# may-/joeys2t

Hardware: AMD Instinct MI355X
Metric: audio frames/sec (train step, 80-mel, 15 s utt, bs32 per GPU) (higher is better)
Workload: dtype bf16; 1 GPU; configs/librispeech_100h.yaml ASR train step on synthetic 16 kHz waveforms; global_batch=32, frames_per_utt=1498, encoder_len=375, lengths=fixed 15 s, vocab=5000, batch_multiplier=1, parallelism=dp1, launch=hipGraph replay

## Files before the change

### include/joeys2t_hip.h

```cpp
#ifndef JOEYS2T_HIP_H
#define JOEYS2T_HIP_H

#include <stdint.h>

#ifdef __cplusplus
extern "C" {
#endif

typedef void* js2t_stream;

enum { JS2T_F32 = 0, JS2T_BF16 = 1, JS2T_FP8_E4M3 = 2  };
enum { JS2T_ACT_NONE = 0, JS2T_ACT_RELU = 1, JS2T_ACT_GELU = 2, JS2T_ACT_SWISH = 3, JS2T_ACT_TANH = 4, JS2T_ACT_HARDSWISH = 5 };
enum { JS2T_OK = 0, JS2T_ERR_INVALID = -1, JS2T_ERR_LAUNCH = -2, JS2T_ERR_UNSUPPORTED = -3 };

int js2t_abi_version(void);
const char* js2t_last_error(void);

typedef struct js2t_gemm_desc {
  int32_t M, N, K;
  int32_t batch, batch_inner;
  int32_t dtype_ab, dtype_c;
  int32_t trans_a, trans_b;
  const void* A; int64_t lda, a_stride_o, a_stride_i;
  const void* B; int64_t ldb, b_stride_o, b_stride_i;
// ... 188 lines not shown
               float log_floor, js2t_stream stream);

int js2t_cmvn_stats(const float* feat, const int64_t* frame_off, int32_t U, int32_t F, float* mean, float* istd,
                    float* fill, int32_t norm_means, int32_t norm_vars, int64_t max_frames, js2t_stream stream);
int64_t js2t_cmvn_stats_workspace(int32_t U, int32_t F);
int js2t_cmvn_stats_ws(const float* feat, const int64_t* frame_off, int32_t U, int32_t F, float* mean, float* istd, float* fill,
                       int32_t norm_means, int32_t norm_vars, int64_t max_frames, double* workspace, js2t_stream stream);

int js2t_feature_finalize(const float* feat, const int64_t* frame_off, const float* mean, const float* istd,
                          const float* fill, const int32_t* masks, void* out, int out_dt, int64_t U, int64_t Tmax,
                          int32_t F, float pad_value, js2t_stream stream);
int js2t_feature_finalize_crop(const float* feat, const int64_t* frame_off, const float* mean, const float* istd,
                               const float* fill, const int32_t* masks, void* out, int out_dt, int64_t U, int64_t Tmax,
                               int32_t F, float pad_value, const int64_t* crop_t, js2t_stream stream);

int js2t_feature_transform(float* feat, const int64_t* frame_off, int32_t U, int32_t F, const float* mean, const float* istd,
                           const float* fill, const int32_t* masks, int32_t n_freq, int32_t n_time, js2t_stream stream);

typedef struct js2t_ctx_s* js2t_ctx;
enum {
  JS2T_CTX_DETERMINISTIC = 0,
  JS2T_CTX_GEMM_P192_MODE = 1,
  JS2T_CTX_GEMM_P192_RING = 2,
  JS2T_CTX_GEMM_WG256_MODE = 3,
  JS2T_CTX_GEMM_PANEL_MODE = 4,
  JS2T_CTX_NKEYS = 5
};
js2t_ctx js2t_ctx_create(void);
void js2t_ctx_destroy(js2t_ctx ctx);
int js2t_ctx_set(js2t_ctx ctx, int32_t key, int32_t value);
// ... 83 lines not shown
```

### joeys2t_amd/csrc/fbank.hip

```cpp
#include "common.hpp"

namespace {

constexpr int FB_WAVES = 4;
constexpr int FB_MAX_FFT = 1024;

__device__ __forceinline__ int find_utt(const int64_t* __restrict__ frame_off, int U, int64_t f) {
  int lo = 0, hi = U;
  while (hi - lo > 1) {
    const int mid = (lo + hi) >> 1;
    if (frame_off[mid] <= f) lo = mid; else hi = mid;
  }
  return lo;
}

__global__ __launch_bounds__(256) void fbank_kernel(const float* __restrict__ wave, const int64_t* __restrict__ sample_off,
                                                    const int64_t* __restrict__ frame_off, int U,
                                                    const float* __restrict__ window, const float* __restrict__ tw_re,
                                                    const float* __restrict__ tw_im, const int32_t* __restrict__ mel_start,
                                                    const int32_t* __restrict__ mel_len, const int32_t* __restrict__ mel_woff,
                                                    const float* __restrict__ mel_w, float* __restrict__ out, int win_len,
                                                    int shift, int n_fft, int log2_fft, int n_mel, float scale,
                                                    float preemph, float log_floor) {
  __shared__ float sre[FB_WAVES][FB_MAX_FFT];
// ... 83 lines not shown
struct cplx { float re, im; };
__device__ __forceinline__ cplx cmul(cplx a, cplx b) { return {a.re * b.re - a.im * b.im, a.re * b.im + a.im * b.re}; }
__device__ __forceinline__ void bfly(cplx& a, cplx& b, cplx w) {
  const cplx d = {a.re - b.re, a.im - b.im};
  a = {a.re + b.re, a.im + b.im};
  b = cmul(d, w);
}
__device__ __forceinline__ void bfly1(cplx& a, cplx& b) {
  const cplx d = {a.re - b.re, a.im - b.im};
  a = {a.re + b.re, a.im + b.im};
  b = d;
}
__device__ __forceinline__ int rev3(int v) { return ((v & 1) << 2) | (v & 2) | ((v >> 2) & 1); }

constexpr int FB5_T1 = 72, FB5_T2 = 9;
constexpr int FB5_MELW = 2048;
__global__ __launch_bounds__(256) void fbank512_kernel(const float* __restrict__ wave, const int64_t* __restrict__ sample_off,
                                                       const int64_t* __restrict__ frame_off, int U,
                                                       const float* __restrict__ window, const float* __restrict__ tw_re,
                                                       const float* __restrict__ tw_im, const int32_t* __restrict__ mel_start,
                                                       const int32_t* __restrict__ mel_len, const int32_t* __restrict__ mel_woff,
                                                       const float* __restrict__ mel_w, float* __restrict__ out, int win_len,
                                                       int shift, int n_mel, float scale, float preemph, float log_floor) {
  __shared__ float2 simg[FB_WAVES][8 * FB5_T1];
  __shared__ float spw[FB_WAVES][256];
  __shared__ float smw[FB5_MELW];
  const int lane = threadIdx.x & 63, w = threadIdx.x >> 6;
  float2* img = simg[w];
  float* pw = spw[w];
  const int n_mel_w = mel_woff[n_mel - 1] + mel_len[n_mel - 1];
  const bool mw_lds = n_mel_w <= FB5_MELW;
  if (mw_lds)
    for (int i = threadIdx.x; i < n_mel_w; i += 256) smw[i] = mel_w[i];
  __syncthreads();
  int mst[2], mln[2], mwo[2];
#pragma unroll
  for (int q = 0; q < 2; ++q) {
    const int mb = lane + 64 * q;
    mst[q] = mb < n_mel ? mel_start[mb] : 0;
    mln[q] = mb < n_mel ? mel_len[mb] : 0;
    mwo[q] = mb < n_mel ? mel_woff[mb] : 0;
  }
  auto tw = [&](int t) -> cplx { return {tw_re[t], tw_im[t]}; };
  const int r = lane & 7;
  cplx w1[4], w2[2], w3, w4[4], w5[2], w6;
#pragma unroll
  for (int j = 0; j < 4; ++j) w1[j] = tw(lane + 64 * j);
#pragma unroll
  for (int j = 0; j < 2; ++j) w2[j] = tw(2 * (lane + 64 * j));
  w3 = tw(4 * lane);
#pragma unroll
  for (int m = 0; m < 4; ++m) w4[m] = tw(8 * (r + 8 * m));
#pragma unroll
  for (int m = 0; m < 2; ++m) w5[m] = tw(16 * (r + 8 * m));
  w6 = tw(32 * r);
  const cplx c8[4] = {{1.f, 0.f}, {0.70710678118654752f, -0.70710678118654752f}, {0.f, -1.f}, {-0.70710678118654752f, -0.70710678118654752f}};
  float win[8];
#pragma unroll
  for (int j = 0; j < 8; ++j) win[j] = lane + 64 * j < win_len ? window[lane + 64 * j] : 0.f;
  const int64_t total = frame_off[U];
  const int64_t n_waves = (int64_t)gridDim.x * FB_WAVES, per = (total + n_waves - 1) / n_waves;
  const int64_t f0 = ((int64_t)blockIdx.x * FB_WAVES + w) * per, f1 = min(total, f0 + per);
  int u = f0 < total ? find_utt(frame_off, U, f0) : 0;
  int64_t u_end = f0 < total ? frame_off[u + 1] : 0, u_beg = f0 < total ? frame_off[u] : 0, s_off = f0 < total ? sample_off[u] : 0;
  auto frame_ptr = [&](int64_t f) -> const float* {
    while (f >= u_end) {
      ++u;
      u_beg = u_end;
      u_end = frame_off[u + 1];
      s_off = sample_off[u];
    }
    return wave + s_off + (f - u_beg) * shift;
  };
  float nxt[8];
  if (f0 < f1) {
    const float* x0 = frame_ptr(f0);
#pragma unroll
    for (int j = 0; j < 8; ++j) nxt[j] = lane + 64 * j < win_len ? x0[lane + 64 * j] : 0.f;
  }
  for (int64_t f = f0; f < f1; ++f) {
    float cur[8], prv[8], sum = 0.f;
#pragma unroll
    for (int j = 0; j < 8; ++j) {
      cur[j] = nxt[j] * scale;
      sum += cur[j];
    }
    if (f + 1 < f1) {
      const float* xn = frame_ptr(f + 1);
#pragma unroll
      for (int j = 0; j < 8; ++j) nxt[j] = lane + 64 * j < win_len ? xn[lane + 64 * j] : 0.f;
    }
#pragma unroll
    for (int j = 0; j < 8; ++j) {
      const float up = __int_as_float(__builtin_amdgcn_update_dpp(0, __float_as_int(cur[j]), 0x138 , 0xf, 0xf, false));
      const int edge = j == 0 ? __builtin_amdgcn_readfirstlane(__float_as_int(cur[0]))
                              : __builtin_amdgcn_readlane(__float_as_int(cur[j > 0 ? j - 1 : 0]), 63);
      prv[j] = lane == 0 ? __int_as_float(edge) : up;
    }
    const float mean = wave_sum(sum) / (float)win_len;
    cplx a[8];
#pragma unroll
    for (int j = 0; j < 8; ++j) a[j] = {lane + 64 * j < win_len ? ((cur[j] - mean) - preemph * (prv[j] - mean)) * win[j] : 0.f, 0.f};
#pragma unroll
    for (int j = 0; j < 4; ++j) bfly(a[j], a[j + 4], w1[j]);
#pragma unroll
    for (int hlf = 0; hlf < 8; hlf += 4)
#pragma unroll
      for (int j = 0; j < 2; ++j) bfly(a[hlf + j], a[hlf + j + 2], w2[j]);
#pragma unroll
    for (int j = 0; j < 8; j += 2) bfly(a[j], a[j + 1], w3);
#pragma unroll
    for (int j = 0; j < 8; ++j) img[j * FB5_T1 + lane] = make_float2(a[j].re, a[j].im);
    asm volatile("s_waitcnt lgkmcnt(0)" ::: "memory");
    const int jp = lane >> 3;
#pragma unroll
    for (int m = 0; m < 8; ++m) {
      const float2 v = img[jp * FB5_T1 + r + 8 * m];
      a[m] = {v.x, v.y};
    }
    asm volatile("s_waitcnt lgkmcnt(0)" ::: "memory");
#pragma unroll
    for (int m = 0; m < 4; ++m) bfly(a[m], a[m + 4], w4[m]);
#pragma unroll
    for (int hlf = 0; hlf < 8; hlf += 4)
#pragma unroll
      for (int m = 0; m < 2; ++m) bfly(a[hlf + m], a[hlf + m + 2], w5[m]);
#pragma unroll
    for (int m = 0; m < 8; m += 2) bfly(a[m], a[m + 1], w6);
#pragma unroll
    for (int m = 0; m < 8; ++m) img[(8 * jp + m) * FB5_T2 + r] = make_float2(a[m].re, a[m].im);
    asm volatile("s_waitcnt lgkmcnt(0)" ::: "memory");
#pragma unroll
    for (int q = 0; q < 8; ++q) {
      const float2 v = img[lane * FB5_T2 + q];
      a[q] = {v.x, v.y};
    }
#pragma unroll
    for (int q = 0; q < 4; ++q) bfly(a[q], a[q + 4], c8[q]);
#pragma unroll
    for (int hlf = 0; hlf < 8; hlf += 4) {
      bfly1(a[hlf], a[hlf + 2]);
      bfly(a[hlf + 1], a[hlf + 3], c8[2]);
    }
#pragma unroll
    for (int q = 0; q < 8; q += 2) bfly1(a[q], a[q + 1]);
    const int mm = lane & 7, base = 8 * rev3(mm) + rev3(jp);
#pragma unroll
    for (int q = 0; q < 8; q += 2) pw[64 * rev3(q) + base] = a[q].re * a[q].re + a[q].im * a[q].im;
    asm volatile("s_waitcnt lgkmcnt(0)" ::: "memory");
#pragma unroll
    for (int q = 0; q < 2; ++q) {
      const int mb = lane + 64 * q;
      if (mb < n_mel) {
        const float* wt = mw_lds ? smw + mwo[q] : mel_w + mwo[q];
        const float* pp = pw + mst[q];
        float e0 = 0.f, e1 = 0.f, e2 = 0.f, e3 = 0.f;
        int k = 0;
        for (; k + 4 <= mln[q]; k += 4) {
          e0 += pp[k] * wt[k];
          e1 += pp[k + 1] * wt[k + 1];
          e2 += pp[k + 2] * wt[k + 2];
          e3 += pp[k + 3] * wt[k + 3];
        }
        for (; k < mln[q]; ++k) e0 += pp[k] * wt[k];
        out[f * n_mel + mb] = __logf(fmaxf((e0 + e1) + (e2 + e3), log_floor));
      }
    }
    for (int mb = lane + 128; mb < n_mel; mb += 64) {
      const int st = mel_start[mb], ln = mel_len[mb];
      const float* wt = mel_w + mel_woff[mb];
      float e = 0.f;
      for (int k = 0; k < ln; ++k) e += pw[st + k] * wt[k];
      out[f * n_mel + mb] = __logf(fmaxf(e, log_floor));
    }
    asm volatile("s_waitcnt lgkmcnt(0)" ::: "memory");
  }
}

constexpr int CM_GROUPS = 12;
constexpr int CM_SPLIT = 8;
__global__ void cmvn_partial_kernel(const float* __restrict__ feat, const int64_t* __restrict__ frame_off, int F, double* __restrict__ part,
                                    int64_t max_frames) {
  extern __shared__ double sh[];
  const int u = blockIdx.x, p = blockIdx.y;
  const int64_t t0 = frame_off[u], T = max_frames > 0 ? min(frame_off[u + 1] - t0, max_frames) : frame_off[u + 1] - t0;
  const int64_t per = (T + CM_SPLIT - 1) / CM_SPLIT, ta = min(T, p * per), tb = min(T, ta + per);
  const int c = threadIdx.x % F, gi = threadIdx.x / F;
  double s = 0.0, q = 0.0;
// ... 101 lines not shown
    float v = t < crop ? pad_value : 0.f;
    if (t < T) {
      v = feat[(t0 + t) * F + c];
      if (mean) v = (v - mean[u * F + c]) * istd[u * F + c];
      if (masks) {
        const int32_t* m = masks + u * 8;
        const bool hit = (m[1] > 0 && c >= m[0] && c < m[0] + m[1]) || (m[3] > 0 && c >= m[2] && c < m[2] + m[3]) ||
                         (m[5] > 0 && t >= m[4] && t < m[4] + m[5]) || (m[7] > 0 && t >= m[6] && t < m[6] + m[7]);
        if (hit) v = fill[u];
      }
    }
    io<TO>::st(out + i, v);
  }
}

__global__ void feature_transform_kernel(float* __restrict__ feat, const int64_t* __restrict__ frame_off, int F,
                                         const float* __restrict__ mean, const float* __restrict__ istd,
                                         const float* __restrict__ fill, const int32_t* __restrict__ masks, int n_freq, int n_time) {
  const int u = blockIdx.y;
  const int64_t t0 = frame_off[u], n = (frame_off[u + 1] - t0) * F;
  const int32_t* m = masks ? masks + (int64_t)u * 2 * (n_freq + n_time) : nullptr;
  for (int64_t i = blockIdx.x * (int64_t)blockDim.x + threadIdx.x; i < n; i += (int64_t)gridDim.x * blockDim.x) {
    const int64_t t = i / F;
    const int c = (int)(i - t * F);
    float v = feat[t0 * F + i];
    if (mean) v = (v - mean[(int64_t)u * F + c]) * istd[(int64_t)u * F + c];
    if (m) {
      bool hit = false;
      for (int k = 0; k < n_freq; ++k) hit = hit || (m[2 * k + 1] > 0 && c >= m[2 * k] && c < m[2 * k] + m[2 * k + 1]);
      for (int k = n_freq; k < n_freq + n_time; ++k) hit = hit || (m[2 * k + 1] > 0 && t >= m[2 * k] && t < m[2 * k] + m[2 * k + 1]);
// ... 95 lines not shown
  int64_t g = (U * Tmax * F + 255) / 256;
  if (g > 8192) g = 8192;
  if (out_dt == JS2T_F32)
    hipLaunchKernelGGL((feature_finalize_kernel<float>), dim3((unsigned)g), dim3(256), 0, (hipStream_t)stream, feat, frame_off,
                       mean, istd, fill, masks, (float*)out, U, Tmax, F, pad_value, crop_t);
  else if (out_dt == JS2T_BF16)
    hipLaunchKernelGGL((feature_finalize_kernel<uint16_t>), dim3((unsigned)g), dim3(256), 0, (hipStream_t)stream, feat,
                       frame_off, mean, istd, fill, masks, (uint16_t*)out, U, Tmax, F, pad_value, crop_t);
  else {
    js2t_set_error("feature_finalize: bad dtype");
    return JS2T_ERR_INVALID;
  }
  JS2T_LAUNCH_CHECK();
  return JS2T_OK;
}
```

### joeys2t_amd/data_augmentation.py

```python
import ctypes as C
import math
from typing import Optional, Sequence

import numpy as np
import torch

from joeys2t_amd import ops
from joeys2t_amd._lib import check, lib

_p, _stream = ops._p, ops._stream


class SpecAugment:

    def __init__(self, freq_mask_n: int = 2, freq_mask_f: int = 27, time_mask_n: int = 2, time_mask_t: int = 40,
                 time_mask_p: float = 1.0, mask_value: Optional[float] = None):
        self.freq_mask_n, self.freq_mask_f = freq_mask_n, freq_mask_f
        self.time_mask_n, self.time_mask_t, self.time_mask_p = time_mask_n, time_mask_t, time_mask_p
        self.mask_value = mask_value

    @property
    def slots(self):
        return max(2, self.freq_mask_n), max(2, self.time_mask_n)

# ... 21 lines not shown

    def __repr__(self):
        return (f"{self.__class__.__name__}(freq_mask_n={self.freq_mask_n}, freq_mask_f={self.freq_mask_f}, "
                f"time_mask_n={self.time_mask_n}, time_mask_t={self.time_mask_t}, time_mask_p={self.time_mask_p})")


class CMVN:

    def __init__(self, norm_means: bool = True, norm_vars: bool = True, before: bool = True):
        self.norm_means, self.norm_vars, self.before = norm_means, norm_vars, before

    def __repr__(self):
        return f"{self.__class__.__name__}(norm_means={self.norm_means}, norm_vars={self.norm_vars}, before={self.before})"


def finalize_features(feat: torch.Tensor, frame_off: torch.Tensor, frames: Sequence[int], *, cmvn: Optional[CMVN],
                      specaugment: Optional[SpecAugment], out_dtype=torch.float32, pad_value: float = 1.0,
                      max_length: Optional[int] = None, masks_dev: Optional[torch.Tensor] = None, t_pad: Optional[int] = None,
                      crop_t: Optional[torch.Tensor] = None):
    ops._dev(feat, frame_off)
    U, F = len(frames), feat.shape[1]
    dev = feat.device
    eff = [min(int(t), max_length) if max_length else int(t) for t in frames]
    Tmax = max(eff) if t_pad is None else int(t_pad)
    mean = istd = fill = masks = None
    fused = ((cmvn is None or cmvn.before) and (specaugment is None or specaugment.fused) and
             not (specaugment is not None and cmvn is None and specaugment.mask_value is None))
    if not fused:
        if masks_dev is not None or crop_t is not None:
            raise NotImplementedError("graph-replayed batches (masks_dev / crop_t) take the fused front-end: CMVN before SpecAugment, "
                                      "at most two masks of each kind")
        return _finalize_general(feat, frame_off, eff, cmvn, specaugment, out_dtype, pad_value, max_length, Tmax)
    if cmvn is not None:
        mean = torch.empty((U, F), dtype=torch.float32, device=dev)
        istd = torch.empty((U, F), dtype=torch.float32, device=dev)
        fill = torch.empty((U, ), dtype=torch.float32, device=dev)
        ws = torch.empty((int(lib().js2t_cmvn_stats_workspace(C.c_int32(U), C.c_int32(F))), ), dtype=torch.float64, device=dev)
        check(lib().js2t_cmvn_stats_ws(_p(feat), _p(frame_off), C.c_int32(U), C.c_int32(F), _p(mean), _p(istd), _p(fill),
                                       C.c_int32(int(cmvn.norm_means)), C.c_int32(int(cmvn.norm_vars)),
                                       C.c_int64(int(max_length) if max_length else 0), _p(ws), _stream()),
              "js2t_cmvn_stats_ws")
    if specaugment is not None:
        if masks_dev is not None:
            masks = masks_dev
        else:
            m = np.stack([specaugment.draw(t, F) for t in eff])
            masks = torch.from_numpy(m).to(dev)
        if specaugment.mask_value is not None:
            fill = torch.full((U, ), float(specaugment.mask_value), dtype=torch.float32, device=dev)
    out = torch.empty((U, Tmax, F), dtype=out_dtype, device=dev)
    check(lib().js2t_feature_finalize_crop(_p(feat), _p(frame_off), _p(mean), _p(istd), _p(fill), _p(masks), _p(out),
                                           ops.dt_code(out), C.c_int64(U), C.c_int64(Tmax), C.c_int32(F), C.c_float(pad_value),
                                           _p(crop_t), _stream()), "js2t_feature_finalize")
    return out, eff


def _stats(feat, frame_off, U, F, norm_means, norm_vars, max_length):
    dev = feat.device
    mean = torch.empty((U, F), dtype=torch.float32, device=dev)
    istd = torch.empty((U, F), dtype=torch.float32, device=dev)
    fill = torch.empty((U, ), dtype=torch.float32, device=dev)
    check(lib().js2t_cmvn_stats(_p(feat), _p(frame_off), C.c_int32(U), C.c_int32(F), _p(mean), _p(istd), _p(fill), C.c_int32(int(norm_means)),
                                C.c_int32(int(norm_vars)), C.c_int64(int(max_length) if max_length else 0), _stream()), "js2t_cmvn_stats")
    return mean, istd, fill

# ... 30 lines not shown
```

### joeys2t_amd/helpers_for_audio.py

```python
import ctypes as C
from pathlib import Path
from typing import Dict, List, Optional, Sequence, Tuple

import numpy as np
import torch

from joeys2t_amd import ops
from joeys2t_amd._lib import check, lib

_p, _stream = ops._p, ops._stream


def get_n_frames(wave_length: int, sample_rate: int) -> int:
    duration_ms = int(wave_length / sample_rate * 1000)
    return int(1 + (duration_ms - 25) / 10)


def _mel(f):
    return 1127.0 * np.log(1.0 + np.asarray(f, dtype=np.float64) / 700.0)


class FbankExtractor:

    def __init__(self, device, sample_rate: int = 16000, n_mel_bins: int = 80, frame_length_ms: float = 25.0,
# ... 25 lines not shown
            starts.append(st), lens.append(ln), woffs.append(len(wts))
            wts.extend(banks[m, st:st + ln].astype(np.float32).tolist())
        dev = self.device
        self.window = torch.tensor(window, dtype=torch.float32, device=dev)
        self.tw_re = torch.tensor(np.cos(ang), dtype=torch.float32, device=dev)
        self.tw_im = torch.tensor(-np.sin(ang), dtype=torch.float32, device=dev)
        self.mel_start = torch.tensor(starts, dtype=torch.int32, device=dev)
        self.mel_len = torch.tensor(lens, dtype=torch.int32, device=dev)
        self.mel_woff = torch.tensor(woffs, dtype=torch.int32, device=dev)
        self.mel_w = torch.tensor(wts if wts else [0.0], dtype=torch.float32, device=dev)
        self._plans = {}

    def n_frames(self, n_samples: int) -> int:
        return 0 if n_samples < self.win_len else 1 + (n_samples - self.win_len) // self.shift

    def batch(self, wave: torch.Tensor, n_samples: Sequence[int], sample_off: Optional[Sequence[int]] = None):
        ops._dev(wave)
        if wave.dtype != torch.float32 or not wave.is_contiguous():
            raise ops.Js2tError("fbank: waveform buffer must be contiguous float32")
        U = len(n_samples)
        if sample_off is None:
            stride = wave.shape[-1] if wave.dim() == 2 else 0
            sample_off = [u * stride for u in range(U)]
        if wave.numel() < max(o + n for o, n in zip(sample_off, n_samples)):
            raise ops.Js2tError("fbank: waveform buffer shorter than sample_off + n_samples")
        key = (tuple(int(n) for n in n_samples), tuple(int(o) for o in sample_off))
        plan = self._plans.get(key)
        if plan is None:
            frames = [self.n_frames(int(n)) for n in n_samples]
            foff = np.concatenate([[0], np.cumsum(frames)]).astype(np.int64)
            plan = (frames, torch.tensor(list(sample_off), dtype=torch.int64, device=self.device),
                    torch.tensor(foff, dtype=torch.int64, device=self.device), int(foff[-1]))
            if len(self._plans) > 64:
                self._plans.clear()
            self._plans[key] = plan
        frames, d_soff, d_foff, total = plan
        return self.batch_tables(wave, d_soff, d_foff, U, total), d_foff, frames

    def batch_tables(self, wave: torch.Tensor, d_soff: torch.Tensor, d_foff: torch.Tensor, U: int, total_cap: int) -> torch.Tensor:
        ops._dev(wave, d_soff, d_foff)
        total = int(total_cap)
        feat = torch.empty((total, self.n_mel), dtype=torch.float32, device=self.device)
        check(lib().js2t_fbank(_p(wave), _p(d_soff), _p(d_foff), C.c_int32(U), C.c_int64(total), _p(self.window),
                               _p(self.tw_re), _p(self.tw_im), _p(self.mel_start), _p(self.mel_len), _p(self.mel_woff),
                               _p(self.mel_w), _p(feat), C.c_int32(self.win_len), C.c_int32(self.shift), C.c_int32(self.n_fft),
                               C.c_int32(self.n_mel), C.c_float(2.0**15), C.c_float(self.preemph),
                               C.c_float(float(np.finfo(np.float32).eps)), _stream()), "js2t_fbank")
        return feat


_extractors: Dict[Tuple, FbankExtractor] = {}


def get_extractor(device, sample_rate: int = 16000, n_mel_bins: int = 80) -> FbankExtractor:
    key = (str(device), int(sample_rate), int(n_mel_bins))
    if key not in _extractors:
        _extractors[key] = FbankExtractor(device, sample_rate, n_mel_bins)
# ... 29 lines not shown
```

### joeys2t_amd/tokenizers.py

```python
import re
from typing import List, Optional, Sequence, Tuple, Union

import torch

from joeys2t_amd.data_augmentation import CMVN, SpecAugment, finalize_features
from joeys2t_amd.helpers_for_audio import get_extractor


class SpeechProcessor:
    def __init__(self, level: str = "frame", num_freq: int = 80, normalize: bool = False, max_length: int = -1,
                 min_length: int = -1, sample_rate: int = 16000, **kwargs):
        self.level = level
        self.num_freq = num_freq
        self.normalize = normalize
        self.max_length = max_length
        self.min_length = min_length
        self.sample_rate = sample_rate
        self.specaugment: Optional[SpecAugment] = SpecAugment(**kwargs["specaugment"]) if "specaugment" in kwargs else None
        self.cmvn: Optional[CMVN] = CMVN(**kwargs["cmvn"]) if "cmvn" in kwargs else None

    def keep_mask(self, frames: Sequence[int], is_train: bool) -> List[bool]:
        keep = []
        for t in frames:
            ok = not (self.min_length > t > 0)
            if ok and 0 < self.max_length < t and is_train:
                ok = False
            keep.append(ok)
        return keep

    def draw_masks(self, frames: Sequence[int]):
        import numpy as np
        eff = [min(int(t), self.max_length) if self.max_length > 0 else int(t) for t in frames]
        return np.stack([self.specaugment.draw(t, self.num_freq) for t in eff])

    def batch_from_waveforms(self, wave: torch.Tensor, n_samples: Sequence[int], is_train: bool = False,
                             out_dtype=torch.float32, sample_off: Optional[Sequence[int]] = None,
                             masks_dev: Optional[torch.Tensor] = None) -> Tuple[torch.Tensor, List[int]]:
        ex = get_extractor(wave.device, self.sample_rate, self.num_freq)
        feat, frame_off, frames = ex.batch(wave, n_samples, sample_off)
        sa = self.specaugment if is_train else None
        return finalize_features(feat, frame_off, frames, cmvn=self.cmvn, specaugment=sa, out_dtype=out_dtype,
                                 max_length=self.max_length if self.max_length > 0 else None, masks_dev=masks_dev)

    def batch_from_tables(self, wave: torch.Tensor, d_soff: torch.Tensor, d_foff: torch.Tensor, n_utts: int, t_pad: int,
                          crop_t: torch.Tensor, is_train: bool = True, out_dtype=torch.float32,
                          masks_dev: Optional[torch.Tensor] = None) -> torch.Tensor:
        ex = get_extractor(wave.device, self.sample_rate, self.num_freq)
        feat = ex.batch_tables(wave, d_soff, d_foff, n_utts, n_utts * t_pad)
        sa = self.specaugment if is_train else None
        if sa is not None and masks_dev is None:
            raise ValueError("batch_from_tables: SpecAugment parameters must be supplied in masks_dev")
        out, _ = finalize_features(feat, d_foff, [t_pad] * n_utts, cmvn=self.cmvn, specaugment=sa, out_dtype=out_dtype,
                                   max_length=None, masks_dev=masks_dev, t_pad=t_pad, crop_t=crop_t)
        return out

    def __repr__(self):
        return (f"{self.__class__.__name__}(level={self.level}, normalize={self.normalize}, "
                f"filter_by_length=({self.min_length}, {self.max_length}), specaugment={self.specaugment}, cmvn={self.cmvn})")


_SPACE_RUNS = re.compile("[ \u3000]+")


def remove_extra_spaces(s: str) -> str:
    s = _SPACE_RUNS.sub(" ", s.replace("\u200b", ""))
    for mark in "?!,.:":
        s = s.replace(" " + mark, mark)
    return s.strip()
# ... 142 lines not shown
```

Measured before the change: 4.270 million frames/s.

## Fuse fbank with CMVN partial statistics and fold stats reduction into finalize

```diff
diff --git a/include/joeys2t_hip.h b/include/joeys2t_hip.h
--- a/include/joeys2t_hip.h
+++ b/include/joeys2t_hip.h
@@ -226,6 +226,16 @@
                                const float* fill, const int32_t* masks, void* out, int out_dt, int64_t U, int64_t Tmax,
                                int32_t F, float pad_value, const int64_t* crop_t, js2t_stream stream);
 
+int js2t_frontend_fused(const float* wave, const int64_t* sample_off, const int64_t* frame_off, int32_t U, int64_t total_frames,
+                        const float* window, const float* tw_re, const float* tw_im, const int32_t* mel_start,
+                        const int32_t* mel_len, const int32_t* mel_woff, const float* mel_w, float* out, int32_t win_len,
+                        int32_t shift, int32_t n_fft, int32_t n_mel, float scale, float preemph, float log_floor,
+                        int64_t max_frames, double* part, js2t_stream stream);
+int js2t_feature_finalize_fused(const float* feat, const int64_t* frame_off, const double* part, int32_t norm_means,
+                                int32_t norm_vars, int64_t max_frames, const float* fill, const int32_t* masks, void* out,
+                                int out_dt, int64_t U, int64_t Tmax, int32_t F, float pad_value, const int64_t* crop_t,
+                                float* mean_out, float* istd_out, float* fill_out, js2t_stream stream);
+
 int js2t_feature_transform(float* feat, const int64_t* frame_off, int32_t U, int32_t F, const float* mean, const float* istd,
                            const float* fill, const int32_t* masks, int32_t n_freq, int32_t n_time, js2t_stream stream);
 
diff --git a/joeys2t_amd/csrc/fbank.hip b/joeys2t_amd/csrc/fbank.hip
--- a/joeys2t_amd/csrc/fbank.hip
+++ b/joeys2t_amd/csrc/fbank.hip
@@ -121,7 +121,130 @@
 __device__ __forceinline__ int rev3(int v) { return ((v & 1) << 2) | (v & 2) | ((v >> 2) & 1); }
 
 constexpr int FB5_T1 = 72, FB5_T2 = 9;
+constexpr int FB5_IMG = 8 * FB5_T1;
 constexpr int FB5_MELW = 2048;
+
+struct fb5_lane {
+  cplx w1[4], w2[2], w3, w4[4], w5[2], w6;
+  float win[8];
+  int mst[2], mln[2], mwo[2];
+};
+__device__ __forceinline__ void fb5_lane_init(fb5_lane& k, int lane, const float* __restrict__ window, const float* __restrict__ tw_re,
+                                              const float* __restrict__ tw_im, const int32_t* __restrict__ mel_start,
+                                              const int32_t* __restrict__ mel_len, const int32_t* __restrict__ mel_woff, int win_len,
+                                              int n_mel) {
+#pragma unroll
+  for (int q = 0; q < 2; ++q) {
+    const int mb = lane + 64 * q;
+    k.mst[q] = mb < n_mel ? mel_start[mb] : 0;
+    k.mln[q] = mb < n_mel ? mel_len[mb] : 0;
+    k.mwo[q] = mb < n_mel ? mel_woff[mb] : 0;
+  }
+  auto tw = [&](int t) -> cplx { return {tw_re[t], tw_im[t]}; };
+  const int r = lane & 7;
+#pragma unroll
+  for (int j = 0; j < 4; ++j) k.w1[j] = tw(lane + 64 * j);
+#pragma unroll
+  for (int j = 0; j < 2; ++j) k.w2[j] = tw(2 * (lane + 64 * j));
+  k.w3 = tw(4 * lane);
+#pragma unroll
+  for (int m = 0; m < 4; ++m) k.w4[m] = tw(8 * (r + 8 * m));
+#pragma unroll
+  for (int m = 0; m < 2; ++m) k.w5[m] = tw(16 * (r + 8 * m));
+  k.w6 = tw(32 * r);
+#pragma unroll
+  for (int j = 0; j < 8; ++j) k.win[j] = lane + 64 * j < win_len ? window[lane + 64 * j] : 0.f;
+}
+
+__device__ __forceinline__ void fb5_frame(const fb5_lane& k, const float (&raw)[8], int lane, float2* img, float* pw, const float* wts, int win_len,
+                                          int n_mel, float scale, float preemph, float log_floor, float (&e)[2]) {
+  const cplx c8[4] = {{1.f, 0.f}, {0.70710678118654752f, -0.70710678118654752f}, {0.f, -1.f}, {-0.70710678118654752f, -0.70710678118654752f}};
+  const int r = lane & 7;
+  float cur[8], prv[8], sum = 0.f;
+#pragma unroll
+  for (int j = 0; j < 8; ++j) {
+    cur[j] = raw[j] * scale;
+    sum += cur[j];
+  }
+#pragma unroll
+  for (int j = 0; j < 8; ++j) {
+    const float up = __int_as_float(__builtin_amdgcn_update_dpp(0, __float_as_int(cur[j]), 0x138 , 0xf, 0xf, false));
+    const int edge = j == 0 ? __builtin_amdgcn_readfirstlane(__float_as_int(cur[0]))
+                            : __builtin_amdgcn_readlane(__float_as_int(cur[j > 0 ? j - 1 : 0]), 63);
+    prv[j] = lane == 0 ? __int_as_float(edge) : up;
+  }
+  const float mean = wave_sum(sum) / (float)win_len;
+  cplx a[8];
+#pragma unroll
+  for (int j = 0; j < 8; ++j) a[j] = {lane + 64 * j < win_len ? ((cur[j] - mean) - preemph * (prv[j] - mean)) * k.win[j] : 0.f, 0.f};
+#pragma unroll
+  for (int j = 0; j < 4; ++j) bfly(a[j], a[j + 4], k.w1[j]);
+#pragma unroll
+  for (int hlf = 0; hlf < 8; hlf += 4)
+#pragma unroll
+    for (int j = 0; j < 2; ++j) bfly(a[hlf + j], a[hlf + j + 2], k.w2[j]);
+#pragma unroll
+  for (int j = 0; j < 8; j += 2) bfly(a[j], a[j + 1], k.w3);
+#pragma unroll
+  for (int j = 0; j < 8; ++j) img[j * FB5_T1 + lane] = make_float2(a[j].re, a[j].im);
+  asm volatile("s_waitcnt lgkmcnt(0)" ::: "memory");
+  const int jp = lane >> 3;
+#pragma unroll
+  for (int m = 0; m < 8; ++m) {
+    const float2 v = img[jp * FB5_T1 + r + 8 * m];
+    a[m] = {v.x, v.y};
+  }
+  asm volatile("s_waitcnt lgkmcnt(0)" ::: "memory");
+#pragma unroll
+  for (int m = 0; m < 4; ++m) bfly(a[m], a[m + 4], k.w4[m]);
+#pragma unroll
+  for (int hlf = 0; hlf < 8; hlf += 4)
+#pragma unroll
+    for (int m = 0; m < 2; ++m) bfly(a[hlf + m], a[hlf + m + 2], k.w5[m]);
+#pragma unroll
+  for (int m = 0; m < 8; m += 2) bfly(a[m], a[m + 1], k.w6);
+#pragma unroll
+  for (int m = 0; m < 8; ++m) img[(8 * jp + m) * FB5_T2 + r] = make_float2(a[m].re, a[m].im);
+  asm volatile("s_waitcnt lgkmcnt(0)" ::: "memory");
+#pragma unroll
+  for (int q = 0; q < 8; ++q) {
+    const float2 v = img[lane * FB5_T2 + q];
+    a[q] = {v.x, v.y};
+  }
+  asm volatile("s_waitcnt lgkmcnt(0)" ::: "memory");
+#pragma unroll
+  for (int q = 0; q < 4; ++q) bfly(a[q], a[q + 4], c8[q]);
+#pragma unroll
+  for (int hlf = 0; hlf < 8; hlf += 4) {
+    bfly1(a[hlf], a[hlf + 2]);
+    bfly(a[hlf + 1], a[hlf + 3], c8[2]);
+  }
+#pragma unroll
+  for (int q = 0; q < 8; q += 2) bfly1(a[q], a[q + 1]);
+  const int mm = lane & 7, base = 8 * rev3(mm) + rev3(jp);
+#pragma unroll
+  for (int q = 0; q < 8; q += 2) pw[64 * rev3(q) + base] = a[q].re * a[q].re + a[q].im * a[q].im;
+  asm volatile("s_waitcnt lgkmcnt(0)" ::: "memory");
+#pragma unroll
+  for (int q = 0; q < 2; ++q) {
+    e[q] = 0.f;
+    if (lane + 64 * q < n_mel) {
+      const float* wt = wts + k.mwo[q];
+      const float* pp = pw + k.mst[q];
+      float e0 = 0.f, e1 = 0.f, e2 = 0.f, e3 = 0.f;
+      int i = 0;
+      for (; i + 4 <= k.mln[q]; i += 4) {
+        e0 += pp[i] * wt[i];
+        e1 += pp[i + 1] * wt[i + 1];
+        e2 += pp[i + 2] * wt[i + 2];
+        e3 += pp[i + 3] * wt[i + 3];
+      }
+      for (; i < k.mln[q]; ++i) e0 += pp[i] * wt[i];
+      e[q] = __logf(fmaxf((e0 + e1) + (e2 + e3), log_floor));
+    }
+  }
+}
+
 __global__ __launch_bounds__(256) void fbank512_kernel(const float* __restrict__ wave, const int64_t* __restrict__ sample_off,
                                                        const int64_t* __restrict__ frame_off, int U,
                                                        const float* __restrict__ window, const float* __restrict__ tw_re,
@@ -129,7 +252,7 @@
                                                        const int32_t* __restrict__ mel_len, const int32_t* __restrict__ mel_woff,
                                                        const float* __restrict__ mel_w, float* __restrict__ out, int win_len,
                                                        int shift, int n_mel, float scale, float preemph, float log_floor) {
-  __shared__ float2 simg[FB_WAVES][8 * FB5_T1];
+  __shared__ float2 simg[FB_WAVES][FB5_IMG];
   __shared__ float spw[FB_WAVES][256];
   __shared__ float smw[FB5_MELW];
   const int lane = threadIdx.x & 63, w = threadIdx.x >> 6;
@@ -140,31 +263,8 @@
   if (mw_lds)
     for (int i = threadIdx.x; i < n_mel_w; i += 256) smw[i] = mel_w[i];
   __syncthreads();
-  int mst[2], mln[2], mwo[2];
-#pragma unroll
-  for (int q = 0; q < 2; ++q) {
-    const int mb = lane + 64 * q;
-    mst[q] = mb < n_mel ? mel_start[mb] : 0;
-    mln[q] = mb < n_mel ? mel_len[mb] : 0;
-    mwo[q] = mb < n_mel ? mel_woff[mb] : 0;
-  }
-  auto tw = [&](int t) -> cplx { return {tw_re[t], tw_im[t]}; };
-  const int r = lane & 7;
-  cplx w1[4], w2[2], w3, w4[4], w5[2], w6;
-#pragma unroll
-  for (int j = 0; j < 4; ++j) w1[j] = tw(lane + 64 * j);
-#pragma unroll
-  for (int j = 0; j < 2; ++j) w2[j] = tw(2 * (lane + 64 * j));
-  w3 = tw(4 * lane);
-#pragma unroll
-  for (int m = 0; m < 4; ++m) w4[m] = tw(8 * (r + 8 * m));
-#pragma unroll
-  for (int m = 0; m < 2; ++m) w5[m] = tw(16 * (r + 8 * m));
-  w6 = tw(32 * r);
-  const cplx c8[4] = {{1.f, 0.f}, {0.70710678118654752f, -0.70710678118654752f}, {0.f, -1.f}, {-0.70710678118654752f, -0.70710678118654752f}};
-  float win[8];
-#pragma unroll
-  for (int j = 0; j < 8; ++j) win[j] = lane + 64 * j < win_len ? window[lane + 64 * j] : 0.f;
+  fb5_lane k;
+  fb5_lane_init(k, lane, window, tw_re, tw_im, mel_start, mel_len, mel_woff, win_len, n_mel);
   const int64_t total = frame_off[U];
   const int64_t n_waves = (int64_t)gridDim.x * FB_WAVES, per = (total + n_waves - 1) / n_waves;
   const int64_t f0 = ((int64_t)blockIdx.x * FB_WAVES + w) * per, f1 = min(total, f0 + per);
@@ -186,99 +286,24 @@
     for (int j = 0; j < 8; ++j) nxt[j] = lane + 64 * j < win_len ? x0[lane + 64 * j] : 0.f;
   }
   for (int64_t f = f0; f < f1; ++f) {
-    float cur[8], prv[8], sum = 0.f;
-#pragma unroll
-    for (int j = 0; j < 8; ++j) {
-      cur[j] = nxt[j] * scale;
-      sum += cur[j];
-    }
+    float raw[8], e[2];
+#pragma unroll
+    for (int j = 0; j < 8; ++j) raw[j] = nxt[j];
     if (f + 1 < f1) {
       const float* xn = frame_ptr(f + 1);
 #pragma unroll
       for (int j = 0; j < 8; ++j) nxt[j] = lane + 64 * j < win_len ? xn[lane + 64 * j] : 0.f;
     }
-#pragma unroll
-    for (int j = 0; j < 8; ++j) {
-      const float up = __int_as_float(__builtin_amdgcn_update_dpp(0, __float_as_int(cur[j]), 0x138 , 0xf, 0xf, false));
-      const int edge = j == 0 ? __builtin_amdgcn_readfirstlane(__float_as_int(cur[0]))
-                              : __builtin_amdgcn_readlane(__float_as_int(cur[j > 0 ? j - 1 : 0]), 63);
-      prv[j] = lane == 0 ? __int_as_float(edge) : up;
-    }
-    const float mean = wave_sum(sum) / (float)win_len;
-    cplx a[8];
-#pragma unroll
-    for (int j = 0; j < 8; ++j) a[j] = {lane + 64 * j < win_len ? ((cur[j] - mean) - preemph * (prv[j] - mean)) * win[j] : 0.f, 0.f};
-#pragma unroll
-    for (int j = 0; j < 4; ++j) bfly(a[j], a[j + 4], w1[j]);
-#pragma unroll
-    for (int hlf = 0; hlf < 8; hlf += 4)
-#pragma unroll
-      for (int j = 0; j < 2; ++j) bfly(a[hlf + j], a[hlf + j + 2], w2[j]);
-#pragma unroll
-    for (int j = 0; j < 8; j += 2) bfly(a[j], a[j + 1], w3);
-#pragma unroll
-    for (int j = 0; j < 8; ++j) img[j * FB5_T1 + lane] = make_float2(a[j].re, a[j].im);
-    asm volatile("s_waitcnt lgkmcnt(0)" ::: "memory");
-    const int jp = lane >> 3;
-#pragma unroll
-    for (int m = 0; m < 8; ++m) {
-      const float2 v = img[jp * FB5_T1 + r + 8 * m];
-      a[m] = {v.x, v.y};
-    }
-    asm volatile("s_waitcnt lgkmcnt(0)" ::: "memory");
-#pragma unroll
-    for (int m = 0; m < 4; ++m) bfly(a[m], a[m + 4], w4[m]);
-#pragma unroll
-    for (int hlf = 0; hlf < 8; hlf += 4)
-#pragma unroll
-      for (int m = 0; m < 2; ++m) bfly(a[hlf + m], a[hlf + m + 2], w5[m]);
-#pragma unroll
-    for (int m = 0; m < 8; m += 2) bfly(a[m], a[m + 1], w6);
-#pragma unroll
-    for (int m = 0; m < 8; ++m) img[(8 * jp + m) * FB5_T2 + r] = make_float2(a[m].re, a[m].im);
-    asm volatile("s_waitcnt lgkmcnt(0)" ::: "memory");
-#pragma unroll
-    for (int q = 0; q < 8; ++q) {
-      const float2 v = img[lane * FB5_T2 + q];
-      a[q] = {v.x, v.y};
-    }
-#pragma unroll
-    for (int q = 0; q < 4; ++q) bfly(a[q], a[q + 4], c8[q]);
-#pragma unroll
-    for (int hlf = 0; hlf < 8; hlf += 4) {
-      bfly1(a[hlf], a[hlf + 2]);
-      bfly(a[hlf + 1], a[hlf + 3], c8[2]);
-    }
-#pragma unroll
-    for (int q = 0; q < 8; q += 2) bfly1(a[q], a[q + 1]);
-    const int mm = lane & 7, base = 8 * rev3(mm) + rev3(jp);
-#pragma unroll
-    for (int q = 0; q < 8; q += 2) pw[64 * rev3(q) + base] = a[q].re * a[q].re + a[q].im * a[q].im;
-    asm volatile("s_waitcnt lgkmcnt(0)" ::: "memory");
-#pragma unroll
-    for (int q = 0; q < 2; ++q) {
-      const int mb = lane + 64 * q;
-      if (mb < n_mel) {
-        const float* wt = mw_lds ? smw + mwo[q] : mel_w + mwo[q];
-        const float* pp = pw + mst[q];
-        float e0 = 0.f, e1 = 0.f, e2 = 0.f, e3 = 0.f;
-        int k = 0;
-        for (; k + 4 <= mln[q]; k += 4) {
-          e0 += pp[k] * wt[k];
-          e1 += pp[k + 1] * wt[k + 1];
-          e2 += pp[k + 2] * wt[k + 2];
-          e3 += pp[k + 3] * wt[k + 3];
-        }
-        for (; k < mln[q]; ++k) e0 += pp[k] * wt[k];
-        out[f * n_mel + mb] = __logf(fmaxf((e0 + e1) + (e2 + e3), log_floor));
-      }
-    }
+    fb5_frame(k, raw, lane, img, pw, mw_lds ? smw : mel_w, win_len, n_mel, scale, preemph, log_floor, e);
+#pragma unroll
+    for (int q = 0; q < 2; ++q)
+      if (lane + 64 * q < n_mel) out[f * n_mel + lane + 64 * q] = e[q];
     for (int mb = lane + 128; mb < n_mel; mb += 64) {
       const int st = mel_start[mb], ln = mel_len[mb];
       const float* wt = mel_w + mel_woff[mb];
-      float e = 0.f;
-      for (int k = 0; k < ln; ++k) e += pw[st + k] * wt[k];
-      out[f * n_mel + mb] = __logf(fmaxf(e, log_floor));
+      float ee = 0.f;
+      for (int i = 0; i < ln; ++i) ee += pw[st + i] * wt[i];
+      out[f * n_mel + mb] = __logf(fmaxf(ee, log_floor));
     }
     asm volatile("s_waitcnt lgkmcnt(0)" ::: "memory");
   }
@@ -410,6 +435,172 @@
   }
 }
 
+__global__ __launch_bounds__(64 * CM_GROUPS) void fbank512_cmvn_kernel(
+    const float* __restrict__ wave, const int64_t* __restrict__ sample_off, const int64_t* __restrict__ frame_off,
+    const float* __restrict__ window, const float* __restrict__ tw_re, const float* __restrict__ tw_im,
+    const int32_t* __restrict__ mel_start, const int32_t* __restrict__ mel_len, const int32_t* __restrict__ mel_woff,
+    const float* __restrict__ mel_w, float* __restrict__ out, double* __restrict__ part, int win_len, int shift, int n_mel, float scale,
+    float preemph, float log_floor, int64_t max_frames) {
+  __shared__ float2 simg[CM_GROUPS][FB5_IMG];
+  __shared__ float smw[FB5_MELW];
+  static_assert(sizeof(double) * 2 * CM_GROUPS * 128 <= sizeof(float2) * CM_GROUPS * FB5_IMG, "group sums of 128 bins fit the images");
+  const int lane = threadIdx.x & 63, g = threadIdx.x >> 6, F = n_mel;
+  const int u = blockIdx.x, p = blockIdx.y;
+  float2* img = simg[g];
+  const int n_mel_w = mel_woff[n_mel - 1] + mel_len[n_mel - 1];
+  const bool mw_lds = n_mel_w <= FB5_MELW;
+  if (mw_lds)
+    for (int i = threadIdx.x; i < n_mel_w; i += 64 * CM_GROUPS) smw[i] = mel_w[i];
+  __syncthreads();
+  fb5_lane k;
+  fb5_lane_init(k, lane, window, tw_re, tw_im, mel_start, mel_len, mel_woff, win_len, n_mel);
+  const int64_t t0 = frame_off[u], T_all = frame_off[u + 1] - t0, T = max_frames > 0 ? min(T_all, max_frames) : T_all;
+  const int64_t per = (T + CM_SPLIT - 1) / CM_SPLIT, ta = min(T, p * per), tb = min(T, ta + per);
+  const int64_t te = p == CM_SPLIT - 1 ? T_all : tb;
+  const float* x = wave + sample_off[u];
+  double s[2] = {0.0, 0.0}, sq[2] = {0.0, 0.0};
+  float nxt[8];
+  int64_t t = ta + g;
+  if (t < te) {
+#pragma unroll
+    for (int j = 0; j < 8; ++j) nxt[j] = lane + 64 * j < win_len ? x[t * shift + lane + 64 * j] : 0.f;
+  }
+  for (; t < te; t += CM_GROUPS) {
+    float raw[8], e[2];
+#pragma unroll
+    for (int j = 0; j < 8; ++j) raw[j] = nxt[j];
+    if (t + CM_GROUPS < te) {
+      const float* xn = x + (t + CM_GROUPS) * shift;
+#pragma unroll
+      for (int j = 0; j < 8; ++j) nxt[j] = lane + 64 * j < win_len ? xn[lane + 64 * j] : 0.f;
+    }
+    fb5_frame(k, raw, lane, img, (float*)img, mw_lds ? smw : mel_w, win_len, n_mel, scale, preemph, log_floor, e);
+#pragma unroll
+    for (int q = 0; q < 2; ++q)
+      if (lane + 64 * q < n_mel) {
+        out[(t0 + t) * n_mel + lane + 64 * q] = e[q];
+        if (t < tb) {
+          const double v = e[q];
+          s[q] += v;
+          sq[q] += v * v;
+        }
+      }
+    asm volatile("s_waitcnt lgkmcnt(0)" ::: "memory");
+  }
+  __syncthreads();
+  double* sh = reinterpret_cast<double*>(&simg[0][0]);
+#pragma unroll
+  for (int q = 0; q < 2; ++q)
+    if (lane + 64 * q < F) {
+      sh[g * F + lane + 64 * q] = s[q];
+      sh[(CM_GROUPS + g) * F + lane + 64 * q] = sq[q];
+    }
+  __syncthreads();
+  if ((int)threadIdx.x < F) {
+    const int c = threadIdx.x;
+    double ss = 0.0, qq = 0.0;
+    for (int g2 = 0; g2 < CM_GROUPS; ++g2) {
+      ss += sh[g2 * F + c];
+      qq += sh[(CM_GROUPS + g2) * F + c];
+    }
+    double* o = part + ((int64_t)u * CM_SPLIT + p) * 2 * F;
+    o[c] = ss;
+    o[F + c] = qq;
+  }
+}
+
+template <typename TO, bool VEC>
+__global__ __launch_bounds__(256) void feature_finalize_fused_kernel(const float* __restrict__ feat, const int64_t* __restrict__ frame_off,
+                                                                     const double* __restrict__ part, const float* __restrict__ fill_in,
+                                                                     const int32_t* __restrict__ masks, TO* __restrict__ out, int64_t Tmax,
+                                                                     int F, float pad_value, const int64_t* __restrict__ crop_t,
+                                                                     int norm_means, int norm_vars, int64_t max_frames,
+                                                                     float* __restrict__ mean_out, float* __restrict__ istd_out,
+                                                                     float* __restrict__ fill_out) {
+  __shared__ float smean[256], sistd[256], sfill;
+  __shared__ double norm_mean[256];
+  const int u = blockIdx.y;
+  const int64_t t0 = frame_off[u], T = frame_off[u + 1] - t0, Ts = max_frames > 0 ? min(T, max_frames) : T;
+  const int64_t crop = crop_t ? *crop_t : Tmax;
+  const bool first = blockIdx.x == 0;
+  if ((int)threadIdx.x < F) {
+    const int c = threadIdx.x;
+    double ss = 0.0, qq = 0.0;
+    for (int p = 0; p < CM_SPLIT; ++p) {
+      const double* in = part + ((int64_t)u * CM_SPLIT + p) * 2 * F;
+      ss += in[c];
+      qq += in[F + c];
+    }
+    const float m = Ts > 0 ? (float)(ss / (double)Ts) : 0.f;
+    const float sqm = Ts > 0 ? (float)(qq / (double)Ts) : 0.f;
+    const float var = sqm - m * m;
+    const float is = norm_vars ? 1.f / sqrtf(fmaxf(var, 1e-10f)) : 1.f;
+    smean[c] = norm_means ? m : 0.f;
+    sistd[c] = is;
+    norm_mean[c] = (double)((norm_means ? 0.f : m) * is);
+    if (first && mean_out) mean_out[(int64_t)u * F + c] = norm_means ? m : 0.f;
+    if (first && istd_out) istd_out[(int64_t)u * F + c] = is;
+  }
+  __syncthreads();
+  if (threadIdx.x == 0) {
+    float fl = 0.f;
+    if (fill_in)
+      fl = fill_in[u];
+    else if (masks || (first && fill_out)) {
+      double a = 0.0;
+      for (int i = 0; i < F; ++i) a += norm_mean[i];
+      fl = (float)(a / (double)F);
+    }
+    sfill = fl;
+    if (first && fill_out) fill_out[u] = fl;
+  }
+  __syncthreads();
+  const float fl = sfill;
+  int32_t m[8] = {0, 0, 0, 0, 0, 0, 0, 0};
+  if (masks)
+#pragma unroll
+    for (int i = 0; i < 8; ++i) m[i] = masks[(int64_t)u * 8 + i];
+  auto value = [&](float v, int64_t t, int c) -> float {
+    v = (v - smean[c]) * sistd[c];
+    const bool hit = (m[1] > 0 && c >= m[0] && c < m[0] + m[1]) || (m[3] > 0 && c >= m[2] && c < m[2] + m[3]) ||
+                     (m[5] > 0 && t >= m[4] && t < m[4] + m[5]) || (m[7] > 0 && t >= m[6] && t < m[6] + m[7]);
+    return hit ? fl : v;
+  };
+  TO* o = out + (int64_t)u * Tmax * F;
+  const float* in = feat + t0 * F;
+  if constexpr (VEC) {
+    const int64_t n8 = Tmax * F / 8;
+    for (int64_t i = blockIdx.x * (int64_t)blockDim.x + threadIdx.x; i < n8; i += (int64_t)gridDim.x * blockDim.x) {
+      const int64_t t = i * 8 / F;
+      const int c = (int)(i * 8 - t * F);
+      float v[8];
+      if (t < T) {
+        const float4 lo = *reinterpret_cast<const float4*>(in + i * 8), hi = *reinterpret_cast<const float4*>(in + i * 8 + 4);
+        const float x8[8] = {lo.x, lo.y, lo.z, lo.w, hi.x, hi.y, hi.z, hi.w};
+#pragma unroll
+        for (int j = 0; j < 8; ++j) v[j] = value(x8[j], t, c + j);
+      } else {
+#pragma unroll
+        for (int j = 0; j < 8; ++j) v[j] = t < crop ? pad_value : 0.f;
+      }
+      if constexpr (sizeof(TO) == 4) {
+        *reinterpret_cast<float4*>(o + i * 8) = make_float4(v[0], v[1], v[2], v[3]);
+        *reinterpret_cast<float4*>(o + i * 8 + 4) = make_float4(v[4], v[5], v[6], v[7]);
+      } else {
+        *reinterpret_cast<uint4*>(o + i * 8) =
+            make_uint4(pack_bf16x2(v[0], v[1]), pack_bf16x2(v[2], v[3]), pack_bf16x2(v[4], v[5]), pack_bf16x2(v[6], v[7]));
+      }
+    }
+  } else {
+    const int64_t n = Tmax * F;
+    for (int64_t i = blockIdx.x * (int64_t)blockDim.x + threadIdx.x; i < n; i += (int64_t)gridDim.x * blockDim.x) {
+      const int64_t t = i / F;
+      const int c = (int)(i - t * F);
+      io<TO>::st(o + i, t < T ? value(in[i], t, c) : (t < crop ? pad_value : 0.f));
+    }
+  }
+}
+
 __global__ void feature_transform_kernel(float* __restrict__ feat, const int64_t* __restrict__ frame_off, int F,
                                          const float* __restrict__ mean, const float* __restrict__ istd,
                                          const float* __restrict__ fill, const int32_t* __restrict__ masks, int n_freq, int n_time) {
@@ -535,3 +726,48 @@
   JS2T_LAUNCH_CHECK();
   return JS2T_OK;
 }
+
+extern "C" int js2t_frontend_fused(const float* wave, const int64_t* sample_off, const int64_t* frame_off, int32_t U, int64_t total_frames,
+                                   const float* window, const float* tw_re, const float* tw_im, const int32_t* mel_start,
+                                   const int32_t* mel_len, const int32_t* mel_woff, const float* mel_w, float* out, int32_t win_len,
+                                   int32_t shift, int32_t n_fft, int32_t n_mel, float scale, float preemph, float log_floor,
+                                   int64_t max_frames, double* part, js2t_stream stream) {
+  if (U == 0) return JS2T_OK;
+  JS2T_CHECK(wave && sample_off && frame_off && window && tw_re && tw_im && mel_start && mel_len && mel_woff && mel_w && part,
+             "frontend_fused: null pointer");
+  JS2T_CHECK(out || total_frames == 0, "frontend_fused: null pointer");
+  JS2T_CHECK(n_fft == 512 && win_len > 0 && win_len <= 512 && shift > 0 && n_mel > 0 && n_mel <= 128,
+             "frontend_fused: 512-point frames of at most 128 mel bins (js2t_fbank + js2t_cmvn_stats_ws cover the rest)");
+  hipLaunchKernelGGL(fbank512_cmvn_kernel, dim3((unsigned)U, CM_SPLIT), dim3(64 * CM_GROUPS), 0, (hipStream_t)stream, wave, sample_off,
+                     frame_off, window, tw_re, tw_im, mel_start, mel_len, mel_woff, mel_w, out, part, win_len, shift, n_mel, scale, preemph,
+                     log_floor, max_frames);
+  JS2T_LAUNCH_CHECK();
+  return JS2T_OK;
+}
+
+extern "C" int js2t_feature_finalize_fused(const float* feat, const int64_t* frame_off, const double* part, int32_t norm_means,
+                                           int32_t norm_vars, int64_t max_frames, const float* fill, const int32_t* masks, void* out,
+                                           int out_dt, int64_t U, int64_t Tmax, int32_t F, float pad_value, const int64_t* crop_t,
+                                           float* mean_out, float* istd_out, float* fill_out, js2t_stream stream) {
+  if (U == 0) return JS2T_OK;
+  JS2T_CHECK(feat && frame_off && part, "feature_finalize_fused: null pointer");
+  JS2T_CHECK(out || Tmax == 0, "feature_finalize_fused: null pointer");
+  JS2T_CHECK(F > 0 && F <= 256 && Tmax >= 0, "feature_finalize_fused: 1..256 feature bins supported");
+  JS2T_CHECK(U <= 65535, "feature_finalize_fused: at most 65535 utterances per call");
+  JS2T_CHECK(out_dt == JS2T_F32 || out_dt == JS2T_BF16, "feature_finalize_fused: bad dtype");
+  const bool vec = F % 8 == 0 && (reinterpret_cast<uintptr_t>(feat) | reinterpret_cast<uintptr_t>(out)) % 16 == 0;
+  int64_t gx = cdiv(Tmax * F, vec ? 8 * 512 : 2048);
+  gx = gx < 1 ? 1 : gx > 256 ? 256 : gx;
+  const dim3 grid((unsigned)gx, (unsigned)U);
+#define JS2T_FFF(TO, VEC)                                                                                                            \
+  hipLaunchKernelGGL((feature_finalize_fused_kernel<TO, VEC>), grid, dim3(256), 0, (hipStream_t)stream, feat, frame_off, part, fill, \
+                     masks, (TO*)out, Tmax, F, pad_value, crop_t, norm_means, norm_vars, max_frames, mean_out, istd_out, fill_out)
+  if (out_dt == JS2T_F32) {
+    if (vec) JS2T_FFF(float, true); else JS2T_FFF(float, false);
+  } else {
+    if (vec) JS2T_FFF(uint16_t, true); else JS2T_FFF(uint16_t, false);
+  }
+#undef JS2T_FFF
+  JS2T_LAUNCH_CHECK();
+  return JS2T_OK;
+}
diff --git a/joeys2t_amd/data_augmentation.py b/joeys2t_amd/data_augmentation.py
--- a/joeys2t_amd/data_augmentation.py
+++ b/joeys2t_amd/data_augmentation.py
@@ -59,10 +59,14 @@
         return f"{self.__class__.__name__}(norm_means={self.norm_means}, norm_vars={self.norm_vars}, before={self.before})"
 
 
+def fused_front_end(cmvn: Optional["CMVN"], specaugment: Optional["SpecAugment"]) -> bool:
+    return cmvn is not None and cmvn.before and (specaugment is None or specaugment.fused)
+
+
 def finalize_features(feat: torch.Tensor, frame_off: torch.Tensor, frames: Sequence[int], *, cmvn: Optional[CMVN],
                       specaugment: Optional[SpecAugment], out_dtype=torch.float32, pad_value: float = 1.0,
                       max_length: Optional[int] = None, masks_dev: Optional[torch.Tensor] = None, t_pad: Optional[int] = None,
-                      crop_t: Optional[torch.Tensor] = None):
+                      crop_t: Optional[torch.Tensor] = None, part: Optional[torch.Tensor] = None):
     ops._dev(feat, frame_off)
     U, F = len(frames), feat.shape[1]
     dev = feat.device
@@ -71,12 +75,14 @@
     mean = istd = fill = masks = None
     fused = ((cmvn is None or cmvn.before) and (specaugment is None or specaugment.fused) and
              not (specaugment is not None and cmvn is None and specaugment.mask_value is None))
+    if part is not None and not (fused and cmvn is not None):
+        raise ValueError("finalize_features: partial sums are taken by the fused front end only (fused_front_end)")
     if not fused:
         if masks_dev is not None or crop_t is not None:
             raise NotImplementedError("graph-replayed batches (masks_dev / crop_t) take the fused front-end: CMVN before SpecAugment, "
                                       "at most two masks of each kind")
         return _finalize_general(feat, frame_off, eff, cmvn, specaugment, out_dtype, pad_value, max_length, Tmax)
-    if cmvn is not None:
+    if cmvn is not None and part is None:
         mean = torch.empty((U, F), dtype=torch.float32, device=dev)
         istd = torch.empty((U, F), dtype=torch.float32, device=dev)
         fill = torch.empty((U, ), dtype=torch.float32, device=dev)
@@ -94,6 +100,13 @@
         if specaugment.mask_value is not None:
             fill = torch.full((U, ), float(specaugment.mask_value), dtype=torch.float32, device=dev)
     out = torch.empty((U, Tmax, F), dtype=out_dtype, device=dev)
+    if part is not None:
+        check(lib().js2t_feature_finalize_fused(_p(feat), _p(frame_off), _p(part), C.c_int32(int(cmvn.norm_means)),
+                                                C.c_int32(int(cmvn.norm_vars)), C.c_int64(int(max_length) if max_length else 0),
+                                                _p(fill), _p(masks), _p(out), ops.dt_code(out), C.c_int64(U), C.c_int64(Tmax),
+                                                C.c_int32(F), C.c_float(pad_value), _p(crop_t), None, None, None, _stream()),
+              "js2t_feature_finalize_fused")
+        return out, eff
     check(lib().js2t_feature_finalize_crop(_p(feat), _p(frame_off), _p(mean), _p(istd), _p(fill), _p(masks), _p(out),
                                            ops.dt_code(out), C.c_int64(U), C.c_int64(Tmax), C.c_int32(F), C.c_float(pad_value),
                                            _p(crop_t), _stream()), "js2t_feature_finalize")
diff --git a/joeys2t_amd/helpers_for_audio.py b/joeys2t_amd/helpers_for_audio.py
--- a/joeys2t_amd/helpers_for_audio.py
+++ b/joeys2t_amd/helpers_for_audio.py
@@ -63,7 +63,16 @@
     def n_frames(self, n_samples: int) -> int:
         return 0 if n_samples < self.win_len else 1 + (n_samples - self.win_len) // self.shift
 
-    def batch(self, wave: torch.Tensor, n_samples: Sequence[int], sample_off: Optional[Sequence[int]] = None):
+    @property
+    def fusable(self) -> bool:
+        return self.n_fft == 512 and self.n_mel <= 128
+
+    def new_part(self, U: int) -> torch.Tensor:
+        n = int(lib().js2t_cmvn_stats_workspace(C.c_int32(U), C.c_int32(self.n_mel)))
+        return torch.empty((n, ), dtype=torch.float64, device=self.device)
+
+    def batch(self, wave: torch.Tensor, n_samples: Sequence[int], sample_off: Optional[Sequence[int]] = None,
+              part: Optional[torch.Tensor] = None, max_frames: int = 0):
         ops._dev(wave)
         if wave.dtype != torch.float32 or not wave.is_contiguous():
             raise ops.Js2tError("fbank: waveform buffer must be contiguous float32")
@@ -84,12 +93,22 @@
                 self._plans.clear()
             self._plans[key] = plan
         frames, d_soff, d_foff, total = plan
-        return self.batch_tables(wave, d_soff, d_foff, U, total), d_foff, frames
+        return self.batch_tables(wave, d_soff, d_foff, U, total, part, max_frames), d_foff, frames
 
-    def batch_tables(self, wave: torch.Tensor, d_soff: torch.Tensor, d_foff: torch.Tensor, U: int, total_cap: int) -> torch.Tensor:
+    def batch_tables(self, wave: torch.Tensor, d_soff: torch.Tensor, d_foff: torch.Tensor, U: int, total_cap: int,
+                     part: Optional[torch.Tensor] = None, max_frames: int = 0) -> torch.Tensor:
         ops._dev(wave, d_soff, d_foff)
         total = int(total_cap)
         feat = torch.empty((total, self.n_mel), dtype=torch.float32, device=self.device)
+        if part is not None:
+            ops._dev(part)
+            check(lib().js2t_frontend_fused(_p(wave), _p(d_soff), _p(d_foff), C.c_int32(U), C.c_int64(total), _p(self.window),
+                                            _p(self.tw_re), _p(self.tw_im), _p(self.mel_start), _p(self.mel_len), _p(self.mel_woff),
+                                            _p(self.mel_w), _p(feat), C.c_int32(self.win_len), C.c_int32(self.shift),
+                                            C.c_int32(self.n_fft), C.c_int32(self.n_mel), C.c_float(2.0**15), C.c_float(self.preemph),
+                                            C.c_float(float(np.finfo(np.float32).eps)), C.c_int64(int(max_frames)), _p(part),
+                                            _stream()), "js2t_frontend_fused")
+            return feat
         check(lib().js2t_fbank(_p(wave), _p(d_soff), _p(d_foff), C.c_int32(U), C.c_int64(total), _p(self.window),
                                _p(self.tw_re), _p(self.tw_im), _p(self.mel_start), _p(self.mel_len), _p(self.mel_woff),
                                _p(self.mel_w), _p(feat), C.c_int32(self.win_len), C.c_int32(self.shift), C.c_int32(self.n_fft),
diff --git a/joeys2t_amd/tokenizers.py b/joeys2t_amd/tokenizers.py
--- a/joeys2t_amd/tokenizers.py
+++ b/joeys2t_amd/tokenizers.py
@@ -1,9 +1,10 @@
+import os
 import re
 from typing import List, Optional, Sequence, Tuple, Union
 
 import torch
 
-from joeys2t_amd.data_augmentation import CMVN, SpecAugment, finalize_features
+from joeys2t_amd.data_augmentation import CMVN, SpecAugment, finalize_features, fused_front_end
 from joeys2t_amd.helpers_for_audio import get_extractor
 
 
@@ -33,25 +34,31 @@
         eff = [min(int(t), self.max_length) if self.max_length > 0 else int(t) for t in frames]
         return np.stack([self.specaugment.draw(t, self.num_freq) for t in eff])
 
+    def _fused(self, ex, sa) -> bool:
+        return ex.fusable and fused_front_end(self.cmvn, sa) and os.environ.get("JS2T_FRONTEND_FUSED", "1") != "0"
+
     def batch_from_waveforms(self, wave: torch.Tensor, n_samples: Sequence[int], is_train: bool = False,
                              out_dtype=torch.float32, sample_off: Optional[Sequence[int]] = None,
                              masks_dev: Optional[torch.Tensor] = None) -> Tuple[torch.Tensor, List[int]]:
         ex = get_extractor(wave.device, self.sample_rate, self.num_freq)
-        feat, frame_off, frames = ex.batch(wave, n_samples, sample_off)
         sa = self.specaugment if is_train else None
+        max_length = self.max_length if self.max_length > 0 else None
+        part = ex.new_part(len(n_samples)) if self._fused(ex, sa) else None
+        feat, frame_off, frames = ex.batch(wave, n_samples, sample_off, part=part, max_frames=max_length or 0)
         return finalize_features(feat, frame_off, frames, cmvn=self.cmvn, specaugment=sa, out_dtype=out_dtype,
-                                 max_length=self.max_length if self.max_length > 0 else None, masks_dev=masks_dev)
+                                 max_length=max_length, masks_dev=masks_dev, part=part)
 
     def batch_from_tables(self, wave: torch.Tensor, d_soff: torch.Tensor, d_foff: torch.Tensor, n_utts: int, t_pad: int,
                           crop_t: torch.Tensor, is_train: bool = True, out_dtype=torch.float32,
                           masks_dev: Optional[torch.Tensor] = None) -> torch.Tensor:
         ex = get_extractor(wave.device, self.sample_rate, self.num_freq)
-        feat = ex.batch_tables(wave, d_soff, d_foff, n_utts, n_utts * t_pad)
         sa = self.specaugment if is_train else None
         if sa is not None and masks_dev is None:
             raise ValueError("batch_from_tables: SpecAugment parameters must be supplied in masks_dev")
+        part = ex.new_part(n_utts) if self._fused(ex, sa) else None
+        feat = ex.batch_tables(wave, d_soff, d_foff, n_utts, n_utts * t_pad, part=part)
         out, _ = finalize_features(feat, d_foff, [t_pad] * n_utts, cmvn=self.cmvn, specaugment=sa, out_dtype=out_dtype,
-                                   max_length=None, masks_dev=masks_dev, t_pad=t_pad, crop_t=crop_t)
+                                   max_length=None, masks_dev=masks_dev, t_pad=t_pad, crop_t=crop_t, part=part)
         return out
 
     def __repr__(self):
```

Result: no change. 4.281 million frames/s (median of 6 runs) (+0.2%).
